# seqan/lambda

Measured on AMD Instinct MI355X. Metric: GCUPS (gapped extension, full-rectangle parity mode; pass-1 cells per second of whole step) searchp BLOSUM62, higher is better.
Workload: dtype f16x2 (exact small integers) + int32

## Files before the change

lambda_amd/csrc/lx_ckpt.hip:

```cpp
#include <hip/hip_runtime.h>

#include <algorithm>
#include <cstdio>
#include <cstdlib>

#include "lx_aids.h"
#include "lx_dp_common.h"

namespace lx
{

#ifndef LX_CKPT_EVERY
#define LX_CKPT_EVERY 16
#endif
constexpr int kCkptEvery = LX_CKPT_EVERY;
#ifndef LX_CKPT_UNROLL
#define LX_CKPT_UNROLL 4
#endif
#define LX_CKPT_PRAGMA(x) _Pragma(#x)
#define LX_CKPT_UNROLL_N(n) LX_CKPT_PRAGMA(unroll n)
#define LX_CKPT_UNROLL_PRAGMA LX_CKPT_UNROLL_N(LX_CKPT_UNROLL)
#ifndef LX_BT_TILE_AT
#define LX_BT_TILE_AT 40
#endif
// ... 475 lines not shown
                ec.s_end = grow + 1;
                ec.flags = (gtie ? kEndAmbiguous : 0) | (int32_t)(ovf_tag << kEndOverflowShift);
            }
            p.ends[e] = ec;
            if (p.score_out)
                p.score_out[e] = bad ? -1 : (active ? gbest : 0);
        }
    }
}

template <int G, int C>
__global__ __launch_bounds__(64, LX_BT_WAVES) void ckpt_backtrace_kernel(TraceParams p)
{
    using Lay               = CkptLayout<G, C>;
    using L16               = Ckpt16Layout<G, C>;
    constexpr int kNibDw    = (C + 7) / 8;
    constexpr int kFar      = -(1 << 28);
    static_assert(kCkptEvery == 16, "the diagonal shortcut reads at most 16 residues per sequence");
    __shared__ int8_t   smat4[kAlph * kAlph];
    __shared__ int8_t   smat1n[kAlph * kAlph];
    __shared__ uint32_t tiles[kCkptEvery * kNibDw * 64];
    constexpr int kRecQ  = 10;
    constexpr int kLdsWg = 20 * 1024 - (int)sizeof(uint32_t) * kCkptEvery * kNibDw * 64 - 2 * kAlph * kAlph;
    constexpr int kPool  = LX_BT_POOL < kLdsWg / (16 * kRecQ) ? LX_BT_POOL : kLdsWg / (16 * kRecQ);
    static_assert(kPool >= 0 && kPool <= 64, "pool masks are 64 bits wide");
    __shared__ uint4 pool[kRecQ][kPool > 0 ? kPool : 1];
#ifdef LX_BT_COUNT
    unsigned long long const bt_entry = (unsigned long long)clock64();
#endif
    for (int x = threadIdx.x; x < kAlph * kAlph; x += blockDim.x)
// ... 2 lines not shown
        smat4[x]    = (int8_t)((v < -32 || v > 31) ? -125 : 4 * v + 3);
        smat1n[x]   = (int8_t)(x == kAlph * kAlph - 1 ? 0 : min(-v, 127));
    }
    __syncthreads();
    uint32_t const lane  = threadIdx.x;
    uint64_t       limit = p.n;
    if (p.count_ptr)
    {
        uint64_t const total = *p.count_ptr;
        limit = total > p.chunk_start ? min(p.n, total - p.chunk_start) : 0;
    }
    int const ge = p.sc->ge, g2 = p.sc->g2;
    int const ge4 = 4 * p.sc->ge, go4 = 4 * p.sc->go;
    uint64_t panel_dw = Lay::slot_dwords(p.steps_cap), panel16_dw = L16::slot_dwords(p.steps_cap), bnd_dw = Lay::bnd_dwords(p.steps_cap);

    bool             have = false, blocked = false, done = false, need_col = false, scan = false, c16 = false;
    uint64_t         po = 0;
    uint64_t         pos = 0;
    EndCell          ec{};
    uint32_t const * slot = nullptr;
    uint32_t         oct_mul = G, ck_mul = G * (L16::kCkDw / 4);
    uint64_t         ck16_off = 0;
    uint8_t const *  q = nullptr, * s = nullptr;
    uint8_t *        ops_al = nullptr;
    uint32_t         cap = 0, a0 = 0, apos = 0, acc = 0, n = 0;
    int              lq = 0, ls = 0;
    int              i = 0, j = 0, end_i = 0, end_j = 0;
    int              res_col = C, res_row = 0x7fffffff;
    int              nar_cw = C, nar_j0 = 0x7fffffff, nar_st0 = 0x7fffffff;
    auto locate = [&](int aj, int & st, int & j0, int & cw)
    {
        if (aj >= nar_j0)
        {
            int const jl = aj - nar_j0;
            int const gl = nar_cw == (3 * C + 3) / 4 ? jl / ((3 * C + 3) / 4) : nar_cw == (C + 1) / 2 ? jl / ((C + 1) / 2) : jl / ((C + 3) / 4);
            st = nar_st0 + gl;
// ... 1 lines not shown
            cw = nar_cw;
        }
        else
        {
            st = aj / C;
            j0 = st * C;
            cw = C;
        }
    };
    int              mode = 0;
    int              left = 0;
    int32_t          nm = 0, nx = 0, np = 0, go = 0, gx = 0;
    bool const       rle_mode = p.rle != nullptr;
    uint32_t         run_op = 3, run_len = 0, ncodes = 0;

    auto dec = [](uint32_t bits16) -> int { return (int)(int16_t)bits16; };
    auto expand = [](uint32_t code16) -> uint32_t
    {
        uint32_t const H = code16 & 0x7ffu;
        return H | ((H - (code16 >> 11)) << 16);
    };
    auto bnd_of = [&](uint32_t pn) { return reinterpret_cast<uint4 const *>(slot + (uint64_t)pn * (c16 ? panel16_dw : panel_dw)); };
    auto rowck_of = [&](uint32_t pn)
    {
        return reinterpret_cast<uint4 const *>(slot + (c16 ? (uint64_t)pn * panel16_dw + ck16_off
                                                           : (uint64_t)pn * panel_dw + bnd_dw));
    };
    auto oct16_index = [&](uint32_t o, uint32_t g_) -> uint32_t { return o * oct_mul + g_; };
    auto ck16_index  = [&](uint32_t m_, uint32_t g_, uint32_t x_) -> uint32_t { return m_ * ck_mul + g_ * (L16::kCkDw / 4) + x_; };
    auto rowck_word_addr = [&](uint32_t m, uint32_t st, uint32_t c) -> uint8_t const *
    {
        if (c16)
            return reinterpret_cast<uint8_t const *>(reinterpret_cast<uint16_t const *>(rowck_of(st / G) + ck16_index(m, st % G, c / 8)) + c % 8);
        return reinterpret_cast<uint8_t const *>(reinterpret_cast<uint32_t const *>(rowck_of(st / G) + rowck_quad_index<G, Lay::kCkDw>(m, st % G, c / 4)) + c % 4);
    };
    auto bnd_word_addr = [&](uint32_t st, uint32_t k) -> uint8_t const *
    {
        if (c16)
            return reinterpret_cast<uint8_t const *>(reinterpret_cast<uint16_t const *>(bnd_of(st / G) + oct16_index(k / 8, st % G)) + (k & 7));
        return reinterpret_cast<uint8_t const *>(reinterpret_cast<uint32_t const *>(bnd_of(st / G) + bnd_quad_index<G>(k / 4, st % G)) + (k & 3));
    };
    auto dword_around = [](uint8_t const * a) -> uint32_t
    {
        return *reinterpret_cast<uint32_t const *>(reinterpret_cast<uintptr_t>(a) & ~(uintptr_t)3);
    };
    auto h_of_dword = [&](uint32_t dw, uint32_t upper_half) -> int
    {
        return c16 ? (int)((dw >> (upper_half ? 16 : 0)) & 0x7ffu) : (int)(int16_t)(dw & 0xffffu);
    };
    auto put_byte = [&](uint32_t byte)
    {
        acc |= byte << (8 * (apos & 3));
        if ((apos & 3) == 0)
        {
            if (apos + 3 <= a0 + cap - 1)
                *reinterpret_cast<uint32_t *>(ops_al + apos) = acc;
            else
                for (uint32_t b = 0; b < 4 && apos + b <= a0 + cap - 1; ++b)
                    ops_al[apos + b] = (uint8_t)(acc >> (8 * b));
            acc = 0;
        }
        --apos;
    };
// ... 29 lines not shown
                return;
            oi = sidx;
        }
        pos                = e;
        po                 = p.out_by_pos ? e : oi;
        uint64_t const  se = p.slot_by_src ? oi : e;
        ec                 = p.ends[se];
        Extension const x  = p.ext[e];
        if (ec.score <= 0)
        {
            Hsp out{};
            out.score     = ec.score < 0 ? -1 : 0;
            p.out_hsp[po] = out;
            return;
        }
        c16                = (ec.flags & kEndCompact) != 0;
        uint32_t const ovf = (uint32_t)ec.flags >> kEndOverflowShift;
        slot               = ovf ? p.ovf + (uint64_t)(ovf - 1) * p.ovf_stride : p.trace + se * p.slot_stride;
        uint32_t steps_e   = p.steps_cap;
        if (p.wf_tab && !ovf)
        {
            WfSlots const  t      = p.wf_tab[se / 16];
            uint64_t const stride = (uint64_t)t.panels_cap * (c16 ? L16::slot_dwords(t.steps_cap) : Lay::slot_dwords(t.steps_cap));
            slot                  = ((p.split_n != 0 && se >= p.split_n) ? p.trace2 : p.trace) + t.off_dw + (se % 16) * stride;
            steps_e               = t.steps_cap;
        }
        panel_dw           = Lay::slot_dwords(steps_e);
        panel16_dw         = L16::slot_dwords(steps_e);
        bnd_dw             = Lay::bnd_dwords(steps_e);
        oct_mul            = G;
        ck_mul             = G * (L16::kCkDw / 4);
        ck16_off           = L16::bnd_dwords(steps_e);
        if (!ovf && (ec.flags & kEndWaveSlots))
        {
            constexpr uint32_t kW = 128 / G;
            uint64_t const     w  = se % kW;
            slot     = p.trace + (se - w) * p.slot_stride + w * (G * 4);
            oct_mul  = kW * G;
            ck_mul   = kW * G * (L16::kCkDw / 4);
            ck16_off = (uint64_t)kW * L16::bnd_dwords(steps_e) - w * (G * 4) + w * (G * L16::kCkDw);
        }
        q                  = p.q_res + x.q_off;
        s                  = p.s_res + x.s_off;
        uint8_t * const ops = p.out_ops + (p.ops_off ? p.ops_off[po] : po * p.ops_stride);
        cap                = x.q_len + x.s_len;
        lq                 = (int)x.q_len;
        ls                 = (int)x.s_len;
        i                  = ec.s_end - 1;
        j                  = ec.q_end - 1;
        {
            int const code = (ec.flags >> kEndNarrowShift) & 3;
            int const last = max(1, (lq + G * C - 1) / (G * C)) - 1;
            nar_cw  = narrow_strip_cols(C, code);
            nar_j0  = code ? last * (G * C) : 0x7fffffff;
            nar_st0 = code ? last * G : 0x7fffffff;
// ... 74 lines not shown
            out.num_matches        = nm;
            out.num_mismatches     = nx;
            out.num_positives      = np;
            out.num_gap_opens      = go;
            out.num_gap_extensions = gx;
            out.ops_shift          = rle_mode ? (int32_t)(uint32_t)at : (int32_t)(cap - n);
        }
        p.out_hsp[po] = out;
        if (rle_mode && p.rle_len)
            p.rle_len[pos] = ec.score > 0 ? ncodes : 0u;
        have          = false;
    };

    auto park = [&](uint32_t e)
    {
        uint32_t const flags = (blocked ? 1u : 0u) | (done ? 2u : 0u) | (need_col ? 4u : 0u) | (scan ? 8u : 0u) | (c16 ? 16u : 0u) |
                               ((uint32_t)mode << 5) | (run_op << 7) | (run_len << 9) | (a0 << 16) | ((uint32_t)nar_cw << 18) |
                               ((uint32_t)res_col << 24);
        uint64_t const sp = reinterpret_cast<uintptr_t>(slot), qp = reinterpret_cast<uintptr_t>(q), spp = reinterpret_cast<uintptr_t>(s),
                       op = reinterpret_cast<uintptr_t>(ops_al);
        pool[0][e] = make_uint4(flags, (uint32_t)pos, (uint32_t)po, (uint32_t)ec.score);
        pool[1][e] = make_uint4((uint32_t)sp, (uint32_t)(sp >> 32), oct_mul, ck_mul);
        pool[2][e] = make_uint4((uint32_t)ck16_off, (uint32_t)panel_dw, (uint32_t)panel16_dw, (uint32_t)bnd_dw);
        pool[3][e] = make_uint4((uint32_t)qp, (uint32_t)(qp >> 32), (uint32_t)spp, (uint32_t)(spp >> 32));
        pool[4][e] = make_uint4((uint32_t)op, (uint32_t)(op >> 32), cap, apos);
        pool[5][e] = make_uint4(acc, n, (uint32_t)lq, (uint32_t)ls);
        pool[6][e] = make_uint4((uint32_t)i, (uint32_t)j, (uint32_t)end_i, (uint32_t)end_j);
        pool[7][e] = make_uint4((uint32_t)res_row, (uint32_t)nar_j0, (uint32_t)nar_st0, (uint32_t)left);
        pool[8][e] = make_uint4((uint32_t)nm, (uint32_t)nx, (uint32_t)np, (uint32_t)go);
        pool[9][e] = make_uint4((uint32_t)gx, ncodes, 0u, 0u);
    };
    auto unpark = [&](uint4 const (&r)[kRecQ])
    {
        uint32_t const flags = r[0].x;
        blocked  = (flags & 1u) != 0;
        done     = (flags & 2u) != 0;
        need_col = (flags & 4u) != 0;
        scan     = (flags & 8u) != 0;
        c16      = (flags & 16u) != 0;
        mode     = (int)((flags >> 5) & 3u);
        run_op   = (flags >> 7) & 3u;
        run_len  = (flags >> 9) & 127u;
        a0       = (flags >> 16) & 3u;
        nar_cw   = (int)((flags >> 18) & 63u);
        res_col  = (int)((flags >> 24) & 63u);
        pos      = r[0].y;
        po       = r[0].z;
        ec.score = (int32_t)r[0].w;
        slot     = reinterpret_cast<uint32_t const *>(((uint64_t)r[1].y << 32) | r[1].x);
        oct_mul  = r[1].z;
        ck_mul   = r[1].w;
        ck16_off   = r[2].x;
        panel_dw   = r[2].y;
        panel16_dw = r[2].z;
        bnd_dw     = r[2].w;
        q      = reinterpret_cast<uint8_t const *>(((uint64_t)r[3].y << 32) | r[3].x);
        s      = reinterpret_cast<uint8_t const *>(((uint64_t)r[3].w << 32) | r[3].z);
        ops_al = reinterpret_cast<uint8_t *>(((uint64_t)r[4].y << 32) | r[4].x);
        cap    = r[4].z;
        apos   = r[4].w;
        acc    = r[5].x;
        n      = r[5].y;
        lq     = (int)r[5].z;
        ls     = (int)r[5].w;
        i      = (int)r[6].x;
        j      = (int)r[6].y;
// ... 398 lines not shown
        uint4 const * const rowck = rowck_of((uint32_t)pn);

        int Hp[C], F[C];
        if (m == 0)
        {
#pragma unroll
            for (int c = 0; c < C; ++c)
            {
                Hp[c] = 0;
                F[c]  = 2;
            }
        }
        else
        {
            uint32_t      w[Lay::kCkDw];
            if (c16)
            {
#pragma unroll
                for (int xq = 0; xq < L16::kCkDw / 4; ++xq)
                {
                    uint4 const    v    = rowck[ck16_index((uint32_t)(m - 1), (uint32_t)gl, (uint32_t)xq)];
                    uint32_t const d[4] = {v.x, v.y, v.z, v.w};
#pragma unroll
                    for (int b = 0; b < 4; ++b)
                    {
                        int const c = 2 * (4 * xq + b);
                        if (c < Lay::kCkDw)
                            w[c] = expand(d[b] & 0xffffu);
                        if (c + 1 < Lay::kCkDw)
                            w[c + 1] = expand(d[b] >> 16);
                    }
// ... 24 lines not shown
#pragma unroll
            for (int c = 0; c < C; ++c)
            {
                uint32_t const r = (c < cw && j0 + c < lq) ? ((qd[c >> 2] >> (8 * (c & 3))) & (kAlph - 1)) : (uint32_t)(kAlph - 1);
                qoff2[c >> 1]    = (c & 1) ? (qoff2[c >> 1] | ((r * kAlph) << 16)) : r * kAlph;
            }
        }
        bool const has_left = st > 0;
        int const  gL       = gl > 0 ? gl - 1 : G - 1;
        int const  qshift   = (gl == 0 && has_left) ? G / 4 : 0;
        uint4 const * const bndL = bnd_of((uint32_t)(gl > 0 ? pn : max(pn - 1, 0)));
        auto load_bq = [&](int qd) -> uint4
        {
            if (!has_left || qd + qshift < 0)
                return make_uint4(0, 0, 0, 0);
            if (c16)
            {
                int const   qs = qd + qshift;
                uint2 const v  = reinterpret_cast<uint2 const *>(bndL + oct16_index((uint32_t)qs / 2, (uint32_t)gL))[qs & 1];
                return make_uint4(expand(v.x & 0xffffu), expand(v.x >> 16), expand(v.y & 0xffffu), expand(v.y >> 16));
            }
            return bndL[bnd_quad_index<G>((uint32_t)(qd + qshift), (uint32_t)gL)];
        };
        int const qd0   = k_base / 4;
        uint4     qprev = load_bq(qd0 - 1), qcur = load_bq(qd0);

        uint32_t snext = *reinterpret_cast<unaligned_u32 const *>(s + max(r_base, 0));
        LX_BT_MARK(kBtTileSetup);
#pragma unroll 1
        for (int t = 0; t < kCkptEvery / 4; ++t)
        {
            if (__ballot(r_base + 4 * t <= i) == 0)
                break;
            uint4 const qnext = load_bq(qd0 + t + 1);
            int const      row0 = r_base + 4 * t;
            int const      lb   = max(row0, 0);
            uint32_t const sdw  = snext;
            snext               = *reinterpret_cast<unaligned_u32 const *>(s + max(row0 + 4, 0));
            uint32_t const lw[4] = {qprev.w, qcur.x, qcur.y, qcur.z};
            uint32_t const dw[4] = {qprev.z, qprev.w, qcur.x, qcur.y};
#pragma unroll
            for (int u = 0; u < 4; ++u)
            {
                int const      row = row0 + u;
                uint32_t const tl  = row >= 0 ? (sdw >> (8 * (row - lb))) & (kAlph - 1) : (uint32_t)(kAlph - 1);
                int            E   = (has_left && row >= 0) ? ((4 * dec(lw[u] >> 16)) | 1) : (kFar | 1);
                int            Hd  = (has_left && row > 0) ? 4 * dec(dw[u] & 0xffffu) : 0;
                uint32_t       w[kNibDw];
#pragma unroll
// ... 161 lines not shown
            if (run_tile && lane == 0)
                bt_walk_phases[min(wmax, (uint32_t)kBtWalkBins - 1)] += 1;
        }
#endif
    }
}


uint64_t ckpt_slot_dwords(int cfg, uint32_t steps_cap)
{
    return cfg == 2   ? CkptLayout<16, 13>::slot_dwords(steps_cap)
           : cfg == 3 ? CkptLayout<8, 13>::slot_dwords(steps_cap)
           : cfg == 4 ? CkptLayout<8, 25>::slot_dwords(steps_cap)
           : cfg == 5 ? CkptLayout<8, 11>::slot_dwords(steps_cap)
                      : CkptLayout<8, 19>::slot_dwords(steps_cap);
}

uint64_t ckpt16_slot_dwords(int cfg, uint32_t steps_cap)
{
    return cfg == 2   ? Ckpt16Layout<16, 13>::slot_dwords(steps_cap)
           : cfg == 3 ? Ckpt16Layout<8, 13>::slot_dwords(steps_cap)
           : cfg == 4 ? Ckpt16Layout<8, 25>::slot_dwords(steps_cap)
           : cfg == 5 ? Ckpt16Layout<8, 11>::slot_dwords(steps_cap)
                      : Ckpt16Layout<8, 19>::slot_dwords(steps_cap);
}

template <int G, int C>
static hipError_t launch_ckpt_forward_cfg(TraceParams const & p, hipStream_t stream)
{
    using Geo = ScoreGeo<G, C>;
// ... 137 lines not shown
```

lambda_amd/csrc/lx_device.h:

```cpp
#pragma once
#include <stdint.h>

namespace lx
{

constexpr int kAlph    = 32;
constexpr int kNegPad  = -100;
constexpr int kMaxTraceRows = 1 << 22;
constexpr int kNegInf  = -(1 << 28);

struct ScoringDev
{
    int32_t alph;
    int32_t go;
    int32_t ge;
    int32_t g2;
    int8_t  mat[kAlph * kAlph];
    int8_t  mat_adj[kAlph * kAlph];
    int8_t  mat_trace[kAlph * kAlph];
    int32_t trace_ok;
    int32_t  smax;
    int32_t  b8_ok;
    int32_t  reserved;
    int16_t  rowmax[kAlph];
// ... 60 lines not shown
    int32_t const *    band_diag;
};

struct EndCell
{
    int32_t score;
    int32_t q_end;
    int32_t s_end;
    int32_t flags;
};
constexpr int32_t kEndAmbiguous = 1;
constexpr int32_t kEndCompact      = 2;
constexpr int     kEndOverflowShift = 8;
constexpr int     kEndNarrowShift   = 2;
constexpr int32_t kEndWaveSlots     = 16;
__host__ __device__ constexpr int narrow_strip_cols(int C, int code) { return code == 0 ? C : code == 1 ? (3 * C + 3) / 4 : code == 2 ? (C + 1) / 2 : (C + 3) / 4; }
constexpr int kNarrowest = 3;
__host__ __device__ constexpr int narrow_code_for(int C, int G, int rem)
{
    return rem <= G * ((C + 3) / 4) ? 3 : rem <= G * ((C + 1) / 2) ? 2 : rem <= G * ((3 * C + 3) / 4) ? 1 : 0;
}

constexpr int      kC16MaxGap = 31;
template <int G, int C>
struct Ckpt16Layout
{
    static constexpr int kCkDw = ((C + 1) / 2 + 3) / 4 * 4;
    __host__ __device__ static constexpr uint64_t bnd_dwords(uint32_t steps_cap) { return (uint64_t)steps_cap / 2 * G; }
    __host__ __device__ static constexpr uint64_t slot_dwords(uint32_t steps_cap)
    {
        return bnd_dwords(steps_cap) + (uint64_t)(steps_cap / 16) * G * kCkDw;
    }
    __host__ __device__ static constexpr uint32_t bnd_oct_index(uint32_t o, uint32_t g) { return o * G + g; }
    __host__ __device__ static constexpr uint32_t rowck_quad_index(uint32_t m, uint32_t g, uint32_t x)
    {
        return (m * G + g) * (kCkDw / 4) + x;
    }
};

struct TraceParams
{
    uint8_t const *    q_res;
    uint8_t const *    s_res;
    Extension const *  ext;
    uint64_t           n;
    ScoringDev const * sc;
    uint32_t *         trace;
    uint64_t           slot_stride;
    uint32_t           steps_cap;
    uint32_t           panels_cap;
    EndCell *          ends;
// ... 98 lines not shown
```

lambda_amd/csrc/lx_handle.cpp:

```cpp
#include "lx_internal.h"

namespace
{
thread_local std::string g_create_error;
}

lx::DevAids const & lx::dev_aids()
{
    static DevAids const aids = []()
    {
        auto num = [](char const * name, long long dflt) -> long long
        {
            char const * e = getenv(name);
            return e && *e ? atoll(e) : dflt;
        };
        auto set = [](char const * name) { return getenv(name) != nullptr; };
        DevAids a{};
        a.host_threads    = (unsigned)std::max(0ll, num("LX_HOST_THREADS", 0));
        a.mq_no_wide      = set("LX_MQ_NO_WIDE");
        a.mq_merge_below  = (uint64_t)std::max(0ll, num("LX_MQ_MERGE_BELOW", 0));
        a.iterate_on_host = set("LX_ITERATE_ON_HOST");
        a.bt_tile_at      = (int)num("LX_BT_TILE_AT", 0);
        a.bt_refill_at    = (int)num("LX_BT_REFILL_AT", 0);
        a.l2_ranges       = (uint64_t)std::min<long long>(std::max(0ll, num("LX_L2_RANGES", 0)), 64);
// ... 372 lines not shown
    d.b8_ok    = f.b8_ok ? 1 : 0;
    for (int a = 0; a < lx::kAlph; ++a)
        for (int b = 0; b < lx::kAlph; ++b)
        {
            bool const pad = a >= sc->alphabet_size || b >= sc->alphabet_size;
            int const  v   = pad ? 0 : sc->matrix[a * LX_ALPH + b] - sc->gap_open;
            d.mat_b8[a * lx::kAlph + b] = (uint8_t)std::min(std::max(v, 0), 255);
        }
    for (int a = 0; a < lx::kAlph; ++a)
    {
        int rm = 0;
        for (int b = 0; b < lx::kAlph; ++b)
        {
            bool const pad = a >= sc->alphabet_size || b >= sc->alphabet_size;
            int const  v   = pad ? lx::kNegPad : sc->matrix[a * LX_ALPH + b] - sc->gap_extend;
            _Float16 const hv = (_Float16)(float)v;
            uint16_t       bits;
            std::memcpy(&bits, &hv, 2);
            d.mat_h[a * lx::kAlph + b]   = bits;
            d.mat_i16[a * lx::kAlph + b] = (int16_t)v;
            if (!pad)
            {
                rm     = std::max(rm, (int)sc->matrix[a * LX_ALPH + b]);
                d.smax = std::max(d.smax, (int)sc->matrix[a * LX_ALPH + b] - sc->gap_extend);
            }
        }
        d.rowmax[a] = (int16_t)rm;
    }
    int rc = bind(h);
    if (rc)
        return rc;
    LX_HIP(h, hipDeviceSynchronize());
    LX_HIP(h, hipMemcpy(h->sc_dev[slot], &d, sizeof(d), hipMemcpyHostToDevice));
    h->sc_host[slot] = *sc;
// ... 26 lines not shown
```

lambda_amd/csrc/lx_score_f16.hip:

```cpp
#include <hip/hip_runtime.h>

#include "lx_aids.h"
#include "lx_dp_common.h"

namespace lx
{

typedef _Float16 h2 __attribute__((ext_vector_type(2)));

#ifndef LX_F16_UNROLL
#define LX_F16_UNROLL 2
#endif
#ifndef LX_F16_CKPT_WAVES
#define LX_F16_CKPT_WAVES 3
#endif
#define LX_PRAGMA(x) _Pragma(#x)
#define LX_UNROLL(n) LX_PRAGMA(unroll n)

__device__ __forceinline__ h2 hmax3(h2 a, h2 b, h2 c)
{
    return __builtin_elementwise_maximum(__builtin_elementwise_maximum(a, b), c);
}
__device__ __forceinline__ h2 hmax(h2 a, h2 b)
{
    return __builtin_elementwise_maximum(a, b);
}
__device__ __forceinline__ h2 hsplat(float x)
{
    return h2{(_Float16)x, (_Float16)x};
}
__device__ __forceinline__ h2 as_h2(uint32_t x)
{
    return __builtin_bit_cast(h2, x);
}
__device__ __forceinline__ uint32_t as_u32(h2 x)
{
    return __builtin_bit_cast(uint32_t, x);
}

constexpr uint32_t kHalfNegInf2 = 0xfc00fc00u;

constexpr uint32_t kHalfTwoPowMinus24x2 = 0x00010001u;
__device__ __forceinline__ uint32_t c16_pack(h2 value_scaled, h2 diff_scaled)
{
    return (as_u32(diff_scaled) << 11) | as_u32(value_scaled);
}

template <int G, int C>
struct PairGeo
{
    static constexpr int kGroups   = 64 / G;
    static constexpr int kPanel    = G * C;
    static constexpr int kUsedDw   = (C + 1) / 2;
    static constexpr int kLaneDw   = (kUsedDw + 3) & ~3;
    static constexpr int kRowDw    = kLaneDw * G;
};

template <int G, int C, bool CKPT>
__global__ __launch_bounds__(64, (CKPT ? (C > 19 ? 2 : LX_F16_CKPT_WAVES) : 1)) void score_pair_kernel(ScoreParams p)
{
// ... 148 lines not shown
            {
                if (8 * x + 2 * w < nrows)
                {
                    dst[(2 * w) * Geo::kRowDw]     = __builtin_amdgcn_perm(r1[w], r0[w], 0x05040100u);
                    dst[(2 * w + 1) * Geo::kRowDw] = __builtin_amdgcn_perm(r1[w], r0[w], 0x07060302u);
                }
            }
        }
    }
    __builtin_amdgcn_fence(__ATOMIC_RELEASE, "wavefront");
    __builtin_amdgcn_wave_barrier();

    uint32_t const row_base  = (uint32_t)(slot_dw + g * Geo::kLaneDw) * 4u;
    constexpr uint32_t kRowBytes = Geo::kRowDw * 4;

    h2 const GE = hsplat((float)ge), G2 = hsplat((float)sc->g2), NGE = hsplat((float)-ge);
    h2       Z  = hsplat((float)(ge * g));
    h2       Hrow[C], F0[C];
#pragma unroll
    for (int c = 0; c < C; ++c)
    {
        Hrow[c] = Z + GE;
        F0[c]   = Z;
    }
    h2 diag0 = Z + GE;
    h2 sendH = Z + GE;
    h2 sendE = as_h2(kHalfNegInf2);
    h2 recvE = as_h2(kHalfNegInf2);
    h2 best  = hsplat(0.f);
    int      rowA = 0, rowB = 0;
    uint32_t tie  = 0;
    h2 const C24 = as_h2(kHalfTwoPowMinus24x2), NC24 = -C24, GEc = GE * C24;
    h2       nZc = -(Z * C24);
    h2       cmax = as_h2(kHalfNegInf2);
    using Lay = Ckpt16Layout<G, C>;
    constexpr uint32_t kW       = 2 * Geo::kGroups;
    constexpr bool     wslots   = CKPT;
    uint32_t * const   waveBase = CKPT ? p.ckpt + (uint64_t)blockIdx.x * kW * p.ckpt_stride : nullptr;
    uint32_t * const   slotA    = !CKPT ? nullptr : wslots ? waveBase + (2 * grp) * (G * 4) : p.ckpt + (actA ? eA : p.n) * p.ckpt_stride;
    uint32_t * const   slotB    = !CKPT ? nullptr : wslots ? waveBase + (2 * grp + 1) * (G * 4) : p.ckpt + (actB ? eB : p.n) * p.ckpt_stride;
    uint32_t const     octMul   = wslots ? kW * G : G;
    uint32_t const     ckMul    = (wslots ? kW * G : G) * (Lay::kCkDw / 4);
    uint32_t * const stage = lds + ((Geo::kGroups + share_g - 1) / share_g) * (nrows * Geo::kRowDw) + lane;

    auto step = [&](uint32_t tA, uint32_t tB, int slot8)
    {
        uint4 const * ra = reinterpret_cast<uint4 const *>(reinterpret_cast<char const *>(lds) + row_base + tA * kRowBytes);
        uint4 const * rb = reinterpret_cast<uint4 const *>(reinterpret_cast<char const *>(lds) + row_base + tB * kRowBytes);
        uint32_t      pa[Geo::kLaneDw], pb[Geo::kLaneDw];
#pragma unroll
        for (int x = 0; x < (Geo::kUsedDw + 3) / 4; ++x)
        {
            if (4 * x + 2 >= Geo::kUsedDw)
            {
                uint2 const va = *reinterpret_cast<uint2 const *>(ra + x), vb = *reinterpret_cast<uint2 const *>(rb + x);
                pa[4 * x] = va.x; pa[4 * x + 1] = va.y;
                pb[4 * x] = vb.x; pb[4 * x + 1] = vb.y;
// ... 26 lines not shown
            h2 const A         = h + G2;
            F0[c]              = hmax3(F0[c], A, ZN);
            Ecur               = hmax(Ecur, A) + GE;
            Hrow[c]            = h;
            if (c & 1)
                rowmax = hmax3(rowmax, Hrow[c - 1], h);
        }
        if (C & 1)
            rowmax = hmax(rowmax, h);
        sendH = h;
        sendE = Ecur;
        h2 const cand = rowmax - Z;
        if constexpr (CKPT)
        {
            cmax = hmax(cmax, cand);
            h2 const hc           = h * C24;
            stage[slot8 * 64]     = c16_pack(hc + nZc, __builtin_elementwise_fma(Ecur, NC24, hc));
            nZc                   = nZc + GEc;
        }
        else
            best = hmax(best, cand);
        Z = ZN;
    };
    auto flush_codes = [&](int k0)
    {
        if constexpr (CKPT)
        {
            uint32_t cw[8];
#pragma unroll
            for (int u = 0; u < 8; ++u)
                cw[u] = stage[u * 64];
            uint32_t const oi = ((uint32_t)k0 / 8) * octMul + (uint32_t)g;
            reinterpret_cast<uint4 *>(slotA)[oi] = make_uint4(__builtin_amdgcn_perm(cw[1], cw[0], 0x05040100u), __builtin_amdgcn_perm(cw[3], cw[2], 0x05040100u),
                                                              __builtin_amdgcn_perm(cw[5], cw[4], 0x05040100u), __builtin_amdgcn_perm(cw[7], cw[6], 0x05040100u));
            reinterpret_cast<uint4 *>(slotB)[oi] = make_uint4(__builtin_amdgcn_perm(cw[1], cw[0], 0x07060302u), __builtin_amdgcn_perm(cw[3], cw[2], 0x07060302u),
                                                              __builtin_amdgcn_perm(cw[5], cw[4], 0x07060302u), __builtin_amdgcn_perm(cw[7], cw[6], 0x07060302u));
        }
    };
    auto book = [&](int k0)
    {
        if constexpr (CKPT)
        {
            h2 const       nb   = hmax(best, cmax);
            uint32_t const rose = as_u32(nb) ^ as_u32(best), met = as_u32(cmax) ^ as_u32(best);
            bool const     gtA = (rose & 0xffffu) != 0, gtB = (rose >> 16) != 0;
            bool const     eqA = (met & 0xffffu) == 0, eqB = (met >> 16) == 0;
            int const last = k0 + 3 - g;
            rowA = gtA ? last : rowA;
            rowB = gtB ? last : rowB;
            tie  = (gtA ? (tie & ~1u) : (tie | (eqA ? 1u : 0u)));
            tie  = (gtB ? (tie & ~2u) : (tie | (eqB ? 2u : 0u)));
// ... 3 lines not shown
    };
    auto chunk_done = [&](int k0)
    {
        if constexpr (CKPT)
        {
#ifndef LX_EXP_NO_FLUSH
            if (k0 & 4)
                flush_codes(k0);
#endif
        }
    };
    auto rowck_store = [&](int k0)
    {
        if constexpr (CKPT)
        {
            h2 const nzic = nZc - GEc, nGEc = -GEc;
            uint32_t code[2 * Lay::kCkDw];
#pragma unroll
            for (int c = 0; c < 2 * Lay::kCkDw; ++c)
                code[c] = c < C ? c16_pack(__builtin_elementwise_fma(Hrow[c < C ? c : 0], C24, nzic),
                                           __builtin_elementwise_fma(Hrow[c < C ? c : 0] - F0[c < C ? c : 0], C24, nGEc))
                                : 0u;
            uint32_t const base0 = (uint32_t)(Lay::bnd_dwords(p.steps_cap) / 4);
            uint4 * const  dA = wslots ? reinterpret_cast<uint4 *>(waveBase) + kW * base0 + (2 * grp) * (G * (Lay::kCkDw / 4)) : reinterpret_cast<uint4 *>(slotA) + base0;
            uint4 * const  dB = wslots ? reinterpret_cast<uint4 *>(waveBase) + kW * base0 + (2 * grp + 1) * (G * (Lay::kCkDw / 4)) : reinterpret_cast<uint4 *>(slotB) + base0;
#pragma unroll
            for (int x = 0; x < Lay::kCkDw / 4; ++x)
            {
                uint32_t wa[4], wb[4];
#pragma unroll
                for (int b = 0; b < 4; ++b)
                {
                    int const c = 2 * (4 * x + b);
                    wa[b]       = __builtin_amdgcn_perm(code[c + 1], code[c], 0x05040100u);
                    wb[b]       = __builtin_amdgcn_perm(code[c + 1], code[c], 0x07060302u);
                }
                uint32_t const qi = ((uint32_t)(k0 + 3) / 16) * ckMul + (uint32_t)g * (Lay::kCkDw / 4) + (uint32_t)x;
                dA[qi] = make_uint4(wa[0], wa[1], wa[2], wa[3]);
                dB[qi] = make_uint4(wb[0], wb[1], wb[2], wb[3]);
            }
        }
    };

    uint32_t const lscA = (uint32_t)max(lsA, 1) - 1u, lscB = (uint32_t)max(lsB, 1) - 1u;
    auto fetch_checked = [&](int k0, uint32_t (&ta)[4], uint32_t (&tb)[4])
    {
#pragma unroll
        for (int u = 0; u < 4; ++u)
        {
            uint32_t const i = (uint32_t)(k0 + u - g);
            ta[u]            = sA[min(i, lscA)];
            tb[u]            = sB[min(i, lscB)];
        }
    };
// ... 68 lines not shown
    }
    if (steps & 4)
        flush_codes(steps);
    if (steps & 15)
        book(steps - 4);

    if constexpr (!CKPT)
    {
#pragma unroll
        for (int off = G / 2; off >= 1; off >>= 1)
            best = hmax(best, as_h2((uint32_t)__shfl_xor((int)as_u32(best), off * kGs)));

        if (is_first)
        {
            if (actA)
                p.out_score[eA] = (int)(float)best.x;
            if (actB)
                p.out_score[eB] = (int)(float)best.y;
        }
    }
    else
    {
        auto finish = [&](int lbest, int lrow, int ltie, bool act, uint64_t e)
        {
            int gbest = lbest, gstrip = g, grow = lrow, gtie = ltie;
#pragma unroll
            for (int off = 1; off < G; off <<= 1)
            {
                int const  ob = __shfl_xor(gbest, off * kGs), os = __shfl_xor(gstrip, off * kGs), orow = __shfl_xor(grow, off * kGs), ot = __shfl_xor(gtie, off * kGs);
                bool const take = ob > gbest || (ob == gbest && os < gstrip);
                gbest  = take ? ob : gbest;
                gstrip = take ? os : gstrip;
                grow   = take ? orow : grow;
                gtie   = take ? ot : gtie;
            }
            if (is_first && act)
            {
                EndCell ec{};
                if (gbest > 0)
                {
                    ec.score = gbest;
                    ec.q_end = -(gstrip + 1);
                    ec.s_end = grow + 1;
                    ec.flags = (gtie ? kEndAmbiguous : 0) | kEndCompact | kEndWaveSlots;
                }
                p.ends[e]      = ec;
                p.out_score[e] = gbest;
            }
        };
        finish((int)(float)best.x, rowA, (int)(tie & 1u), actA, eA);
        finish((int)(float)best.y, rowB, (int)((tie >> 1) & 1u), actB, eB);
    }
}

template <int G, int C, bool CKPT = false>
static hipError_t launch_pair_cfg(ScoreParams const & p, hipStream_t stream)
{
    using Geo = PairGeo<G, C>;
    uint64_t const per_wave = 2ull * Geo::kGroups;
    uint64_t const blocks   = (p.n + per_wave - 1) / per_wave;
    if (blocks > 0x7fffffffull)
        return hipErrorInvalidValue;
    bool const   split = p.pair_share > 0 && p.pair_share < Geo::kGroups;
    int const    slots = split ? Geo::kGroups / p.pair_share : 1;
    if (split && slots * p.pair_share != Geo::kGroups)
        return hipErrorInvalidValue;
// ... 77 lines not shown
```

lambda_amd/csrc/lx_step_plan.cpp:

```cpp
#include "lx_step_plan.h"

#include <algorithm>
#include <cstdio>

#include "lx_device.h"

namespace lxi
{

SchemeFacts scheme_facts(lx_scoring const & sc)
{
    SchemeFacts f{};
    f.alph       = sc.alphabet_size;
    f.gap_open   = sc.gap_open;
    f.gap_extend = sc.gap_extend;
    f.trace_ok   = true;
    f.b8_ok      = true;
    f.smax_entry = 0;
    for (int a = 0; a < sc.alphabet_size; ++a)
        for (int b = 0; b < sc.alphabet_size; ++b)
        {
            int const v = sc.matrix[a * LX_ALPH + b];
            if (v - sc.gap_extend < -31 || v - sc.gap_extend > 31)
                f.trace_ok = false;
// ... 298 lines not shown
    int const G = lx::trace_cfg_group(c.cfg);
    c.steps     = steps_for(o.max_slen, G);
    c.stride32  = (uint64_t)c.panels * lx::ckpt_slot_dwords(c.cfg, c.steps);
    bool const g8 = c.cfg == 1 || c.cfg == 3 || c.cfg == 4;
    c.packed      = half_ok && c.panels == 1 && ((g8 && run16) || c.cfg == 2);
    c.wide_compact = half_ok && c.panels > 1 && c.cfg == 1 && run16;
    c.packed       = c.packed || c.wide_compact;
    if (half_ok && c.panels == 1 && (c.cfg == 1 || c.cfg == 3) && !c.packed && o.query_run % 8 == 0 &&
        two_profiles_bytes(pair_cfg_of(c.cfg), nrows) <= pair_lds_limit())
    {
        c.packed = true;
        c.share  = 4;
    }
    if (c.packed)
    {
        c.stride = (uint64_t)c.panels * lx::ckpt16_slot_dwords(c.cfg, c.steps);
        c.runs   = packed_fits(o, c.stride);
        c.may_decline = score_bound(sc, o.max_qlen, c.steps, G) > kCompactMaxScore || c.wide_compact;
        if (c.runs && c.may_decline)
            c.ovf_cap = overflow_slots(o, c);
    }
    else
    {
        c.stride = c.stride32;
        c.runs   = o.n * c.stride * 4 <= o.trace_bytes;
    }
    return c;
}

}

// ... 59 lines not shown
```

lambda_amd/csrc/lx_step_plan.h:

```cpp
#pragma once
#include <cstddef>
#include <cstdint>

#include "../../include/lambda_ext.h"

namespace lx
{
int      score_cfg_panel(int cfg);
int      score_cfg_groups(int cfg);
int      score_cfg_count();
int      score_pair_cfg_for(uint32_t max_qlen);
int      score_pair_cfg_cols(int cfg);
int      score_pair_cfg_for_runs_of_8(uint32_t max_qlen);
int      score_pair_cfg_group(int cfg);
size_t   score_pair_profile_bytes(int cfg, int nrows);
int      trace_cfg_panel(int cfg);
int      trace_cfg_group(int cfg);
int      trace_cfg_words(int cfg);
uint64_t ckpt_slot_dwords(int cfg, uint32_t steps_cap);
uint64_t ckpt16_slot_dwords(int cfg, uint32_t steps_cap);
size_t   sweep_mq_lds_bytes(int trace_cfg, int nrows, int share);
}

namespace lxi
{

struct SchemeFacts
{
    int  alph = 0, gap_open = 0, gap_extend = 0, smax_entry = 0;
    bool trace_ok = false, b8_ok = false;
    int  nrows() const { return (alph + 1 + 3) / 4 * 4; }
};
SchemeFacts scheme_facts(lx_scoring const & sc);

struct ListLimits
// ... 93 lines not shown
```

Before: 6009.

## Store f16 checkpoints as integer-unit halves in paired-lane wave layout

The f16 score kernel now encodes scores as raw integer bit patterns (sign-magnitude units in the half bits) instead of real half values scaled by 2^-24. This drops the multiply and FMA scaling in the checkpoint path and the float conversions at output. Checkpoint words keep both lanes of an h2 pair together in a new CkptPairLayout, so the perm shuffles that split A/B lanes into separate slots go away and each store becomes a plain uint4. The backtrace kernel gains a pair/odd-lane mode that extracts the right 16-bit half with bitfield extracts. The risk is that half-precision max/add on denormal-range bit patterns must stay exact, and the backtrace addressing grows more complex.

Result: faster. 6143 (median of 6 runs) (+2.2%).

```diff
diff --git a/lambda_amd/csrc/lx_ckpt.hip b/lambda_amd/csrc/lx_ckpt.hip
--- a/lambda_amd/csrc/lx_ckpt.hip
+++ b/lambda_amd/csrc/lx_ckpt.hip
@@ -513,6 +513,7 @@
 {
     using Lay               = CkptLayout<G, C>;
     using L16               = Ckpt16Layout<G, C>;
+    using LP                = CkptPairLayout<G, C>;
     constexpr int kNibDw    = (C + 7) / 8;
     constexpr int kFar      = -(1 << 28);
     static_assert(kCkptEvery == 16, "the diagonal shortcut reads at most 16 residues per sequence");
@@ -545,12 +546,22 @@
     int const ge4 = 4 * p.sc->ge, go4 = 4 * p.sc->go;
     uint64_t panel_dw = Lay::slot_dwords(p.steps_cap), panel16_dw = L16::slot_dwords(p.steps_cap), bnd_dw = Lay::bnd_dwords(p.steps_cap);
 
-    bool             have = false, blocked = false, done = false, need_col = false, scan = false, c16 = false;
+    bool             have = false, blocked = false, done = false, need_col = false, scan = false;
     uint64_t         po = 0;
     uint64_t         pos = 0;
     EndCell          ec{};
     uint32_t const * slot = nullptr;
-    uint32_t         oct_mul = G, ck_mul = G * (L16::kCkDw / 4);
+    uint32_t         kind = 0;
+    constexpr uint32_t kKindC16 = 1u, kKindPair = 2u, kKindWave = 4u, kKindOdd = 16u;
+    constexpr uint32_t kW16 = 128 / G;
+    static_assert(LP::bnd_quad_index(0, 8, 0) == kW16 * G, "a pair's two quads of four steps take the room of two windows' groups of eight");
+    auto oct_mul = [&]() -> uint32_t { return (kind & kKindWave) ? kW16 * G : (uint32_t)G; };
+    auto ck_mul  = [&]() -> uint32_t
+    {
+        return (kind & kKindPair)   ? LP::rowck_quad_index(0, 1, 0, 0)
+               : (kind & kKindWave) ? kW16 * G * (L16::kCkDw / 4)
+                                    : (uint32_t)(G * (L16::kCkDw / 4));
+    };
     uint64_t         ck16_off = 0;
     uint8_t const *  q = nullptr, * s = nullptr;
     uint8_t *        ops_al = nullptr;
@@ -582,30 +593,42 @@
     bool const       rle_mode = p.rle != nullptr;
     uint32_t         run_op = 3, run_len = 0, ncodes = 0;
 
+    auto is_c16  = [&]() { return (kind & kKindC16) != 0; };
+    auto is_pair = [&]() { return (kind & kKindPair) != 0; };
     auto dec = [](uint32_t bits16) -> int { return (int)(int16_t)bits16; };
     auto expand = [](uint32_t code16) -> uint32_t
     {
         uint32_t const H = code16 & 0x7ffu;
         return H | ((H - (code16 >> 11)) << 16);
     };
-    auto bnd_of = [&](uint32_t pn) { return reinterpret_cast<uint4 const *>(slot + (uint64_t)pn * (c16 ? panel16_dw : panel_dw)); };
+    auto expand_half = [](uint32_t d, uint32_t sh) -> uint32_t
+    {
+        uint32_t const H = __builtin_amdgcn_ubfe(d, sh, 11u);
+        return H | ((H - __builtin_amdgcn_ubfe(d, sh + 11u, 5u)) << 16);
+    };
+    auto bnd_of = [&](uint32_t pn) { return reinterpret_cast<uint4 const *>(slot + (uint64_t)pn * (is_c16() ? panel16_dw : panel_dw)); };
     auto rowck_of = [&](uint32_t pn)
     {
-        return reinterpret_cast<uint4 const *>(slot + (c16 ? (uint64_t)pn * panel16_dw + ck16_off
+        return reinterpret_cast<uint4 const *>(slot + (is_c16() ? (uint64_t)pn * panel16_dw + ck16_off
                                                            : (uint64_t)pn * panel_dw + bnd_dw));
     };
-    auto oct16_index = [&](uint32_t o, uint32_t g_) -> uint32_t { return o * oct_mul + g_; };
-    auto ck16_index  = [&](uint32_t m_, uint32_t g_, uint32_t x_) -> uint32_t { return m_ * ck_mul + g_ * (L16::kCkDw / 4) + x_; };
+    auto bnd16_index = [&](uint32_t k_, uint32_t g_) -> uint32_t { return (k_ / 8) * oct_mul() + (is_pair() ? ((k_ >> 2) & 1u) * G : 0u) + g_; };
+    auto ck16_index  = [&](uint32_t m_, uint32_t g_, uint32_t x_) -> uint32_t
+    {
+        return m_ * ck_mul() + g_ * (is_pair() ? (uint32_t)LP::kCkQuads : (uint32_t)(L16::kCkDw / 4)) + x_;
+    };
     auto rowck_word_addr = [&](uint32_t m, uint32_t st, uint32_t c) -> uint8_t const *
     {
-        if (c16)
-            return reinterpret_cast<uint8_t const *>(reinterpret_cast<uint16_t const *>(rowck_of(st / G) + ck16_index(m, st % G, c / 8)) + c % 8);
+        if (is_c16())
+            return reinterpret_cast<uint8_t const *>(reinterpret_cast<uint16_t const *>(rowck_of(st / G) + ck16_index(m, st % G, is_pair() ? c / 4 : c / 8))
+                                                     + (is_pair() ? ((c & 3u) << 1) | (kind >> 4) : c & 7u));
         return reinterpret_cast<uint8_t const *>(reinterpret_cast<uint32_t const *>(rowck_of(st / G) + rowck_quad_index<G, Lay::kCkDw>(m, st % G, c / 4)) + c % 4);
     };
     auto bnd_word_addr = [&](uint32_t st, uint32_t k) -> uint8_t const *
     {
-        if (c16)
-            return reinterpret_cast<uint8_t const *>(reinterpret_cast<uint16_t const *>(bnd_of(st / G) + oct16_index(k / 8, st % G)) + (k & 7));
+        if (is_c16())
+            return reinterpret_cast<uint8_t const *>(reinterpret_cast<uint16_t const *>(bnd_of(st / G) + bnd16_index(k, st % G))
+                                                     + (is_pair() ? ((k & 3u) << 1) | (kind >> 4) : k & 7u));
         return reinterpret_cast<uint8_t const *>(reinterpret_cast<uint32_t const *>(bnd_of(st / G) + bnd_quad_index<G>(k / 4, st % G)) + (k & 3));
     };
     auto dword_around = [](uint8_t const * a) -> uint32_t
@@ -614,7 +637,7 @@
     };
     auto h_of_dword = [&](uint32_t dw, uint32_t upper_half) -> int
     {
-        return c16 ? (int)((dw >> (upper_half ? 16 : 0)) & 0x7ffu) : (int)(int16_t)(dw & 0xffffu);
+        return is_c16() ? (int)((dw >> (upper_half ? 16 : 0)) & 0x7ffu) : (int)(int16_t)(dw & 0xffffu);
     };
     auto put_byte = [&](uint32_t byte)
     {
@@ -674,31 +697,40 @@
             p.out_hsp[po] = out;
             return;
         }
-        c16                = (ec.flags & kEndCompact) != 0;
+        bool const c16     = (ec.flags & kEndCompact) != 0;
+        kind               = c16 ? kKindC16 : 0u;
         uint32_t const ovf = (uint32_t)ec.flags >> kEndOverflowShift;
         slot               = ovf ? p.ovf + (uint64_t)(ovf - 1) * p.ovf_stride : p.trace + se * p.slot_stride;
         uint32_t steps_e   = p.steps_cap;
         if (p.wf_tab && !ovf)
         {
             WfSlots const  t      = p.wf_tab[se / 16];
-            uint64_t const stride = (uint64_t)t.panels_cap * (c16 ? L16::slot_dwords(t.steps_cap) : Lay::slot_dwords(t.steps_cap));
+            uint64_t const stride = (uint64_t)t.panels_cap * (is_c16() ? L16::slot_dwords(t.steps_cap) : Lay::slot_dwords(t.steps_cap));
             slot                  = ((p.split_n != 0 && se >= p.split_n) ? p.trace2 : p.trace) + t.off_dw + (se % 16) * stride;
             steps_e               = t.steps_cap;
         }
         panel_dw           = Lay::slot_dwords(steps_e);
         panel16_dw         = L16::slot_dwords(steps_e);
         bnd_dw             = Lay::bnd_dwords(steps_e);
-        oct_mul            = G;
-        ck_mul             = G * (L16::kCkDw / 4);
         ck16_off           = L16::bnd_dwords(steps_e);
         if (!ovf && (ec.flags & kEndWaveSlots))
         {
-            constexpr uint32_t kW = 128 / G;
+            constexpr uint32_t kW = kW16;
             uint64_t const     w  = se % kW;
-            slot     = p.trace + (se - w) * p.slot_stride + w * (G * 4);
-            oct_mul  = kW * G;
-            ck_mul   = kW * G * (L16::kCkDw / 4);
-            ck16_off = (uint64_t)kW * L16::bnd_dwords(steps_e) - w * (G * 4) + w * (G * L16::kCkDw);
+            kind |= kKindWave;
+            if (ec.flags & kEndPairSlots)
+            {
+                uint32_t const pr    = (uint32_t)w / 2;
+                uint32_t const first = LP::bnd_quad_index(pr, 0, 0) * 4;
+                kind |= kKindPair | (((uint32_t)w & 1u) ? kKindOdd : 0u);
+                slot     = p.trace + (se - w) * p.slot_stride + first;
+                ck16_off = (uint64_t)kW * LP::bnd_dwords(steps_e) - first + LP::rowck_quad_index(pr, 0, 0, 0) * 4;
+            }
+            else
+            {
+                slot     = p.trace + (se - w) * p.slot_stride + w * (G * 4);
+                ck16_off = (uint64_t)kW * L16::bnd_dwords(steps_e) - w * (G * 4) + w * (G * L16::kCkDw);
+            }
         }
         q                  = p.q_res + x.q_off;
         s                  = p.s_res + x.s_off;
@@ -803,13 +835,13 @@
 
     auto park = [&](uint32_t e)
     {
-        uint32_t const flags = (blocked ? 1u : 0u) | (done ? 2u : 0u) | (need_col ? 4u : 0u) | (scan ? 8u : 0u) | (c16 ? 16u : 0u) |
+        uint32_t const flags = (blocked ? 1u : 0u) | (done ? 2u : 0u) | (need_col ? 4u : 0u) | (scan ? 8u : 0u) |
                                ((uint32_t)mode << 5) | (run_op << 7) | (run_len << 9) | (a0 << 16) | ((uint32_t)nar_cw << 18) |
                                ((uint32_t)res_col << 24);
         uint64_t const sp = reinterpret_cast<uintptr_t>(slot), qp = reinterpret_cast<uintptr_t>(q), spp = reinterpret_cast<uintptr_t>(s),
                        op = reinterpret_cast<uintptr_t>(ops_al);
         pool[0][e] = make_uint4(flags, (uint32_t)pos, (uint32_t)po, (uint32_t)ec.score);
-        pool[1][e] = make_uint4((uint32_t)sp, (uint32_t)(sp >> 32), oct_mul, ck_mul);
+        pool[1][e] = make_uint4((uint32_t)sp, (uint32_t)(sp >> 32), kind, 0u);
         pool[2][e] = make_uint4((uint32_t)ck16_off, (uint32_t)panel_dw, (uint32_t)panel16_dw, (uint32_t)bnd_dw);
         pool[3][e] = make_uint4((uint32_t)qp, (uint32_t)(qp >> 32), (uint32_t)spp, (uint32_t)(spp >> 32));
         pool[4][e] = make_uint4((uint32_t)op, (uint32_t)(op >> 32), cap, apos);
@@ -826,7 +858,6 @@
         done     = (flags & 2u) != 0;
         need_col = (flags & 4u) != 0;
         scan     = (flags & 8u) != 0;
-        c16      = (flags & 16u) != 0;
         mode     = (int)((flags >> 5) & 3u);
         run_op   = (flags >> 7) & 3u;
         run_len  = (flags >> 9) & 127u;
@@ -837,8 +868,7 @@
         po       = r[0].z;
         ec.score = (int32_t)r[0].w;
         slot     = reinterpret_cast<uint32_t const *>(((uint64_t)r[1].y << 32) | r[1].x);
-        oct_mul  = r[1].z;
-        ck_mul   = r[1].w;
+        kind     = r[1].z;
         ck16_off   = r[2].x;
         panel_dw   = r[2].y;
         panel16_dw = r[2].z;
@@ -1267,7 +1297,21 @@
         else
         {
             uint32_t      w[Lay::kCkDw];
-            if (c16)
+            if (is_pair())
+            {
+                uint32_t const sh = kind & kKindOdd;
+#pragma unroll
+                for (int xq = 0; xq < LP::kCkQuads; ++xq)
+                {
+                    uint4 const    v    = rowck[ck16_index((uint32_t)(m - 1), (uint32_t)gl, (uint32_t)xq)];
+                    uint32_t const d[4] = {v.x, v.y, v.z, v.w};
+#pragma unroll
+                    for (int b = 0; b < 4; ++b)
+                        if (4 * xq + b < Lay::kCkDw)
+                            w[4 * xq + b] = expand_half(d[b], sh);
+                }
+            }
+            else if (is_c16())
             {
 #pragma unroll
                 for (int xq = 0; xq < L16::kCkDw / 4; ++xq)
@@ -1322,10 +1366,16 @@
         {
             if (!has_left || qd + qshift < 0)
                 return make_uint4(0, 0, 0, 0);
-            if (c16)
+            if (is_pair())
+            {
+                uint32_t const sh = kind & kKindOdd;
+                uint4 const    v  = bndL[bnd16_index(4u * (uint32_t)(qd + qshift), (uint32_t)gL)];
+                return make_uint4(expand_half(v.x, sh), expand_half(v.y, sh), expand_half(v.z, sh), expand_half(v.w, sh));
+            }
+            if (is_c16())
             {
                 int const   qs = qd + qshift;
-                uint2 const v  = reinterpret_cast<uint2 const *>(bndL + oct16_index((uint32_t)qs / 2, (uint32_t)gL))[qs & 1];
+                uint2 const v  = reinterpret_cast<uint2 const *>(bndL + bnd16_index(8u * ((uint32_t)qs / 2), (uint32_t)gL))[qs & 1];
                 return make_uint4(expand(v.x & 0xffffu), expand(v.x >> 16), expand(v.y & 0xffffu), expand(v.y >> 16));
             }
             return bndL[bnd_quad_index<G>((uint32_t)(qd + qshift), (uint32_t)gL)];
@@ -1340,7 +1390,7 @@
         {
             if (__ballot(r_base + 4 * t <= i) == 0)
                 break;
-            uint4 const qnext = load_bq(qd0 + t + 1);
+            uint4 const qnext = t + 1 < kCkptEvery / 4 ? load_bq(qd0 + t + 1) : make_uint4(0, 0, 0, 0);
             int const      row0 = r_base + 4 * t;
             int const      lb   = max(row0, 0);
             uint32_t const sdw  = snext;
@@ -1532,6 +1582,15 @@
            : cfg == 4 ? CkptLayout<8, 25>::slot_dwords(steps_cap)
            : cfg == 5 ? CkptLayout<8, 11>::slot_dwords(steps_cap)
                       : CkptLayout<8, 19>::slot_dwords(steps_cap);
+}
+
+uint64_t ckpt_pair_slot_dwords(int cfg, uint32_t steps_cap)
+{
+    return cfg == 2   ? CkptPairLayout<16, 13>::slot_dwords(steps_cap)
+           : cfg == 3 ? CkptPairLayout<8, 13>::slot_dwords(steps_cap)
+           : cfg == 4 ? CkptPairLayout<8, 25>::slot_dwords(steps_cap)
+           : cfg == 5 ? CkptPairLayout<8, 11>::slot_dwords(steps_cap)
+                      : CkptPairLayout<8, 19>::slot_dwords(steps_cap);
 }
 
 uint64_t ckpt16_slot_dwords(int cfg, uint32_t steps_cap)
diff --git a/lambda_amd/csrc/lx_device.h b/lambda_amd/csrc/lx_device.h
--- a/lambda_amd/csrc/lx_device.h
+++ b/lambda_amd/csrc/lx_device.h
@@ -98,6 +98,7 @@
 constexpr int     kEndOverflowShift = 8;
 constexpr int     kEndNarrowShift   = 2;
 constexpr int32_t kEndWaveSlots     = 16;
+constexpr int32_t kEndPairSlots     = 32;
 __host__ __device__ constexpr int narrow_strip_cols(int C, int code) { return code == 0 ? C : code == 1 ? (3 * C + 3) / 4 : code == 2 ? (C + 1) / 2 : (C + 3) / 4; }
 constexpr int kNarrowest = 3;
 __host__ __device__ constexpr int narrow_code_for(int C, int G, int rem)
@@ -119,6 +120,26 @@
     __host__ __device__ static constexpr uint32_t rowck_quad_index(uint32_t m, uint32_t g, uint32_t x)
     {
         return (m * G + g) * (kCkDw / 4) + x;
+    }
+};
+
+template <int G, int C>
+struct CkptPairLayout
+{
+    static constexpr int kPairs = 64 / G;
+    static constexpr int kCkQuads = (C + 3) / 4;
+    __host__ __device__ static constexpr uint64_t bnd_dwords(uint32_t steps_cap) { return (uint64_t)steps_cap / 2 * G; }
+    __host__ __device__ static constexpr uint64_t slot_dwords(uint32_t steps_cap)
+    {
+        return bnd_dwords(steps_cap) + (uint64_t)(steps_cap / 16) * G * (kCkQuads * 2);
+    }
+    __host__ __device__ static constexpr uint32_t bnd_quad_index(uint32_t pair, uint32_t k, uint32_t g)
+    {
+        return (((k / 8) * kPairs + pair) * 2 + ((k / 4) & 1)) * G + g;
+    }
+    __host__ __device__ static constexpr uint32_t rowck_quad_index(uint32_t pair, uint32_t m, uint32_t g, uint32_t x)
+    {
+        return ((m * kPairs + pair) * G + g) * kCkQuads + x;
     }
 };
 
diff --git a/lambda_amd/csrc/lx_handle.cpp b/lambda_amd/csrc/lx_handle.cpp
--- a/lambda_amd/csrc/lx_handle.cpp
+++ b/lambda_amd/csrc/lx_handle.cpp
@@ -410,10 +410,7 @@
         {
             bool const pad = a >= sc->alphabet_size || b >= sc->alphabet_size;
             int const  v   = pad ? lx::kNegPad : sc->matrix[a * LX_ALPH + b] - sc->gap_extend;
-            _Float16 const hv = (_Float16)(float)v;
-            uint16_t       bits;
-            std::memcpy(&bits, &hv, 2);
-            d.mat_h[a * lx::kAlph + b]   = bits;
+            d.mat_h[a * lx::kAlph + b]   = (uint16_t)(v < 0 ? 0x8000 | -v : v);
             d.mat_i16[a * lx::kAlph + b] = (int16_t)v;
             if (!pad)
             {
diff --git a/lambda_amd/csrc/lx_score_f16.hip b/lambda_amd/csrc/lx_score_f16.hip
--- a/lambda_amd/csrc/lx_score_f16.hip
+++ b/lambda_amd/csrc/lx_score_f16.hip
@@ -25,10 +25,6 @@
 {
     return __builtin_elementwise_maximum(a, b);
 }
-__device__ __forceinline__ h2 hsplat(float x)
-{
-    return h2{(_Float16)x, (_Float16)x};
-}
 __device__ __forceinline__ h2 as_h2(uint32_t x)
 {
     return __builtin_bit_cast(h2, x);
@@ -38,12 +34,20 @@
     return __builtin_bit_cast(uint32_t, x);
 }
 
+__device__ __forceinline__ h2 hunits(int n)
+{
+    uint32_t const m = (uint32_t)min(n < 0 ? -n : n, 2047);
+    return as_h2((n < 0 ? 0x8000u | m : m) * 0x10001u);
+}
+__device__ __forceinline__ int units_of(uint32_t half_bits)
+{
+    return (int)(half_bits & 0x7fffu);
+}
 constexpr uint32_t kHalfNegInf2 = 0xfc00fc00u;
 
-constexpr uint32_t kHalfTwoPowMinus24x2 = 0x00010001u;
-__device__ __forceinline__ uint32_t c16_pack(h2 value_scaled, h2 diff_scaled)
-{
-    return (as_u32(diff_scaled) << 11) | as_u32(value_scaled);
+__device__ __forceinline__ uint32_t c16_pack(h2 value, h2 diff)
+{
+    return (as_u32(diff) << 11) | as_u32(value);
 }
 
 template <int G, int C>
@@ -222,8 +226,8 @@
     uint32_t const row_base  = (uint32_t)(slot_dw + g * Geo::kLaneDw) * 4u;
     constexpr uint32_t kRowBytes = Geo::kRowDw * 4;
 
-    h2 const GE = hsplat((float)ge), G2 = hsplat((float)sc->g2), NGE = hsplat((float)-ge);
-    h2       Z  = hsplat((float)(ge * g));
+    h2 const GE = hunits(ge), G2 = hunits(sc->g2), NGE = hunits(-ge);
+    h2       Z  = hunits(ge * g);
     h2       Hrow[C], F0[C];
 #pragma unroll
     for (int c = 0; c < C; ++c)
@@ -235,20 +239,18 @@
     h2 sendH = Z + GE;
     h2 sendE = as_h2(kHalfNegInf2);
     h2 recvE = as_h2(kHalfNegInf2);
-    h2 best  = hsplat(0.f);
+    h2 best  = hunits(0);
     int      rowA = 0, rowB = 0;
     uint32_t tie  = 0;
-    h2 const C24 = as_h2(kHalfTwoPowMinus24x2), NC24 = -C24, GEc = GE * C24;
-    h2       nZc = -(Z * C24);
     h2       cmax = as_h2(kHalfNegInf2);
-    using Lay = Ckpt16Layout<G, C>;
+    using Lay = CkptPairLayout<G, C>;
     constexpr uint32_t kW       = 2 * Geo::kGroups;
-    constexpr bool     wslots   = CKPT;
-    uint32_t * const   waveBase = CKPT ? p.ckpt + (uint64_t)blockIdx.x * kW * p.ckpt_stride : nullptr;
-    uint32_t * const   slotA    = !CKPT ? nullptr : wslots ? waveBase + (2 * grp) * (G * 4) : p.ckpt + (actA ? eA : p.n) * p.ckpt_stride;
-    uint32_t * const   slotB    = !CKPT ? nullptr : wslots ? waveBase + (2 * grp + 1) * (G * 4) : p.ckpt + (actB ? eB : p.n) * p.ckpt_stride;
-    uint32_t const     octMul   = wslots ? kW * G : G;
-    uint32_t const     ckMul    = (wslots ? kW * G : G) * (Lay::kCkDw / 4);
+    uint4 * const      waveBase = CKPT ? reinterpret_cast<uint4 *>(p.ckpt + (uint64_t)blockIdx.x * kW * p.ckpt_stride) : nullptr;
+    uint4 * const      bndBase  = CKPT ? waveBase + Lay::bnd_quad_index((uint32_t)grp, 0, (uint32_t)g) : nullptr;
+    uint4 * const      ckBase   = CKPT ? waveBase + kW * (uint32_t)(Lay::bnd_dwords(p.steps_cap) / 4) + Lay::rowck_quad_index((uint32_t)grp, 0, (uint32_t)g, 0) : nullptr;
+    constexpr uint32_t kOctMul  = Lay::bnd_quad_index(0, 8, 0);
+    constexpr uint32_t kHalfOct = Lay::bnd_quad_index(0, 4, 0);
+    constexpr uint32_t kCkMul   = Lay::rowck_quad_index(0, 1, 0, 0);
     uint32_t * const stage = lds + ((Geo::kGroups + share_g - 1) / share_g) * (nrows * Geo::kRowDw) + lane;
 
     auto step = [&](uint32_t tA, uint32_t tB, int slot8)
@@ -305,9 +307,7 @@
         if constexpr (CKPT)
         {
             cmax = hmax(cmax, cand);
-            h2 const hc           = h * C24;
-            stage[slot8 * 64]     = c16_pack(hc + nZc, __builtin_elementwise_fma(Ecur, NC24, hc));
-            nZc                   = nZc + GEc;
+            stage[slot8 * 64] = c16_pack(h - Z, h - Ecur);
         }
         else
             best = hmax(best, cand);
@@ -321,11 +321,9 @@
 #pragma unroll
             for (int u = 0; u < 8; ++u)
                 cw[u] = stage[u * 64];
-            uint32_t const oi = ((uint32_t)k0 / 8) * octMul + (uint32_t)g;
-            reinterpret_cast<uint4 *>(slotA)[oi] = make_uint4(__builtin_amdgcn_perm(cw[1], cw[0], 0x05040100u), __builtin_amdgcn_perm(cw[3], cw[2], 0x05040100u),
-                                                              __builtin_amdgcn_perm(cw[5], cw[4], 0x05040100u), __builtin_amdgcn_perm(cw[7], cw[6], 0x05040100u));
-            reinterpret_cast<uint4 *>(slotB)[oi] = make_uint4(__builtin_amdgcn_perm(cw[1], cw[0], 0x07060302u), __builtin_amdgcn_perm(cw[3], cw[2], 0x07060302u),
-                                                              __builtin_amdgcn_perm(cw[5], cw[4], 0x07060302u), __builtin_amdgcn_perm(cw[7], cw[6], 0x07060302u));
+            uint4 * const dst = bndBase + ((uint32_t)k0 / 8) * kOctMul;
+            dst[0]        = make_uint4(cw[0], cw[1], cw[2], cw[3]);
+            dst[kHalfOct] = make_uint4(cw[4], cw[5], cw[6], cw[7]);
         }
     };
     auto book = [&](int k0)
@@ -359,30 +357,19 @@
     {
         if constexpr (CKPT)
         {
-            h2 const nzic = nZc - GEc, nGEc = -GEc;
-            uint32_t code[2 * Lay::kCkDw];
-#pragma unroll
-            for (int c = 0; c < 2 * Lay::kCkDw; ++c)
-                code[c] = c < C ? c16_pack(__builtin_elementwise_fma(Hrow[c < C ? c : 0], C24, nzic),
-                                           __builtin_elementwise_fma(Hrow[c < C ? c : 0] - F0[c < C ? c : 0], C24, nGEc))
-                                : 0u;
-            uint32_t const base0 = (uint32_t)(Lay::bnd_dwords(p.steps_cap) / 4);
-            uint4 * const  dA = wslots ? reinterpret_cast<uint4 *>(waveBase) + kW * base0 + (2 * grp) * (G * (Lay::kCkDw / 4)) : reinterpret_cast<uint4 *>(slotA) + base0;
-            uint4 * const  dB = wslots ? reinterpret_cast<uint4 *>(waveBase) + kW * base0 + (2 * grp + 1) * (G * (Lay::kCkDw / 4)) : reinterpret_cast<uint4 *>(slotB) + base0;
-#pragma unroll
-            for (int x = 0; x < Lay::kCkDw / 4; ++x)
-            {
-                uint32_t wa[4], wb[4];
+            h2 const      zi  = Z + GE;
+            uint4 * const dst = ckBase + ((uint32_t)(k0 + 3) / 16) * kCkMul;
+#pragma unroll
+            for (int x = 0; x < Lay::kCkQuads; ++x)
+            {
+                uint32_t code[4];
 #pragma unroll
                 for (int b = 0; b < 4; ++b)
                 {
-                    int const c = 2 * (4 * x + b);
-                    wa[b]       = __builtin_amdgcn_perm(code[c + 1], code[c], 0x05040100u);
-                    wb[b]       = __builtin_amdgcn_perm(code[c + 1], code[c], 0x07060302u);
+                    int const c = 4 * x + b;
+                    code[b]     = c < C ? c16_pack(Hrow[c < C ? c : 0] - zi, (Hrow[c < C ? c : 0] - F0[c < C ? c : 0]) + NGE) : 0u;
                 }
-                uint32_t const qi = ((uint32_t)(k0 + 3) / 16) * ckMul + (uint32_t)g * (Lay::kCkDw / 4) + (uint32_t)x;
-                dA[qi] = make_uint4(wa[0], wa[1], wa[2], wa[3]);
-                dB[qi] = make_uint4(wb[0], wb[1], wb[2], wb[3]);
+                dst[x] = make_uint4(code[0], code[1], code[2], code[3]);
             }
         }
     };
@@ -481,9 +468,9 @@
         if (is_first)
         {
             if (actA)
-                p.out_score[eA] = (int)(float)best.x;
+                p.out_score[eA] = units_of(as_u32(best));
             if (actB)
-                p.out_score[eB] = (int)(float)best.y;
+                p.out_score[eB] = units_of(as_u32(best) >> 16);
         }
     }
     else
@@ -509,14 +496,14 @@
                     ec.score = gbest;
                     ec.q_end = -(gstrip + 1);
                     ec.s_end = grow + 1;
-                    ec.flags = (gtie ? kEndAmbiguous : 0) | kEndCompact | kEndWaveSlots;
+                    ec.flags = (gtie ? kEndAmbiguous : 0) | kEndCompact | kEndWaveSlots | kEndPairSlots;
                 }
                 p.ends[e]      = ec;
                 p.out_score[e] = gbest;
             }
         };
-        finish((int)(float)best.x, rowA, (int)(tie & 1u), actA, eA);
-        finish((int)(float)best.y, rowB, (int)((tie >> 1) & 1u), actB, eB);
+        finish(units_of(as_u32(best)), rowA, (int)(tie & 1u), actA, eA);
+        finish(units_of(as_u32(best) >> 16), rowB, (int)((tie >> 1) & 1u), actB, eB);
     }
 }
 
diff --git a/lambda_amd/csrc/lx_step_plan.cpp b/lambda_amd/csrc/lx_step_plan.cpp
--- a/lambda_amd/csrc/lx_step_plan.cpp
+++ b/lambda_amd/csrc/lx_step_plan.cpp
@@ -336,7 +336,7 @@
     }
     if (c.packed)
     {
-        c.stride = (uint64_t)c.panels * lx::ckpt16_slot_dwords(c.cfg, c.steps);
+        c.stride = c.wide_compact ? (uint64_t)c.panels * lx::ckpt16_slot_dwords(c.cfg, c.steps) : lx::ckpt_pair_slot_dwords(c.cfg, c.steps);
         c.runs   = packed_fits(o, c.stride);
         c.may_decline = score_bound(sc, o.max_qlen, c.steps, G) > kCompactMaxScore || c.wide_compact;
         if (c.runs && c.may_decline)
diff --git a/lambda_amd/csrc/lx_step_plan.h b/lambda_amd/csrc/lx_step_plan.h
--- a/lambda_amd/csrc/lx_step_plan.h
+++ b/lambda_amd/csrc/lx_step_plan.h
@@ -19,6 +19,7 @@
 int      trace_cfg_words(int cfg);
 uint64_t ckpt_slot_dwords(int cfg, uint32_t steps_cap);
 uint64_t ckpt16_slot_dwords(int cfg, uint32_t steps_cap);
+uint64_t ckpt_pair_slot_dwords(int cfg, uint32_t steps_cap);
 size_t   sweep_mq_lds_bytes(int trace_cfg, int nrows, int share);
 }
 
```
